# lavaman131/dinov2.cpp

Hardware: AMD Instinct MI355X
Metric: images/sec (518x518), ViT-L/14 fp16 (higher is better)
Workload: dtype f16; 1 GPU; dinov2-large (ViT-L/14, 4 registers) f16 GGUF, 518x518, batch=32 per GPU, classify head, random-init weights; global_batch=32, parallelism=dp1

## Files before the change

dinov2.cpp_amd/csrc/gemm4.hip:

```cpp
#include <cstdio>
#include <type_traits>
#include <utility>

#include "device_types.h"
#include "gemm_epilogue.h"
#include "kernels.h"

namespace dinov2 {

template <int... Is, class F>
static __device__ __forceinline__ void static_for_impl(std::integer_sequence<int, Is...>, F&& f) {
    (f(std::integral_constant<int, Is>{}), ...);
}
template <int N, class F>
static __device__ __forceinline__ void static_for(F&& f) {
    static_for_impl(std::make_integer_sequence<int, N>{}, static_cast<F&&>(f));
}

#define DINO4_MFMA_F16(ACC, W, X) asm volatile("v_mfma_f32_16x16x32_f16 %0, %1, %2, %0" : "+a"(ACC) : "v"(W), "v"(X))
#define DINO4_MFMA_F16_Z(ACC, W, X) asm volatile("v_mfma_f32_16x16x32_f16 %0, %1, %2, 0" : "=a"(ACC) : "v"(W), "v"(X))
#define DINO4_MFMA_BF16(ACC, W, X) asm volatile("v_mfma_f32_16x16x32_bf16 %0, %1, %2, %0" : "+a"(ACC) : "v"(W), "v"(X))
#define DINO4_MFMA_BF16_Z(ACC, W, X) asm volatile("v_mfma_f32_16x16x32_bf16 %0, %1, %2, 0" : "=a"(ACC) : "v"(W), "v"(X))
#define DINO4_DSR(DST, ADDR, OFF) asm volatile("ds_read_b128 %0, %1 offset:%2" : "=v"(DST) : "v"(ADDR), "n"(OFF))
#define DINO4_GLDS(VOFF, SBASE, LDSBASE, IMM)                                                                                   \
    asm volatile("s_add_u32 m0, %2, %3\n\ts_nop 0\n\tglobal_load_lds_dwordx4 %0, %1" ::"v"(VOFF), "s"(SBASE), "s"(LDSBASE), "n"(IMM) \
                 : "memory", "scc")

__device__ unsigned long long g_clk4[CLK_SLOTS * 4];
hipError_t gemm4_clock_probe_read(unsigned long long* out) {
    return hipMemcpyFromSymbol(out, HIP_SYMBOL(g_clk4), sizeof(unsigned long long) * CLK_SLOTS * 4);
}

constexpr int G4_PA = 39, G4_PB = 103;

#ifdef DINO_GEMM4_PROF
__device__ unsigned long long g_gemm4_prof[256 * 4];
#define DINO4_GP_DECL unsigned long long gp_t = 0, gp_r = 0, gp_acc[4] = {0, 0, 0, 0};
#define DINO4_GP_START { gp_t = __builtin_readcyclecounter(); gp_r = __builtin_amdgcn_s_memrealtime(); }
#define DINO4_GP(i) { const unsigned long long t__ = __builtin_readcyclecounter(); gp_acc[i] += t__ - gp_t; gp_t = t__; }
#define DINO4_GP_TILE { gp_acc[2] += 1; const unsigned long long r__ = __builtin_amdgcn_s_memrealtime(); gp_acc[3] += r__ - gp_r; gp_r = r__; }
#define DINO4_GP_FLUSH if (threadIdx.x == 0) for (int i__ = 0; i__ < 4; ++i__) g_gemm4_prof[blockIdx.x * 4 + i__] += gp_acc[i__];
#else
#define DINO4_GP_DECL
#define DINO4_GP_START
#define DINO4_GP(i)
#define DINO4_GP_TILE
#define DINO4_GP_FLUSH
#endif

template <typename T, int EPI, int NI>
static __device__ __forceinline__ void gemm4_body(const GemmArgs& p, char* smem) {
#pragma clang fp contract(off)
    using E = Elem<T>;
    using vec4 = typename E::vec4;
    constexpr bool F16 = std::is_same<T, _Float16>::value;
    constexpr bool LNC = EPI == EPI_QKV_LN || EPI == EPI_GELU_LN || EPI == EPI_SWIGLU_LN;
    constexpr int EB = EPI == EPI_RESID_LN ? EPI_RESID : EPI == EPI_QKV_LN ? EPI_QKV : EPI == EPI_GELU_LN ? EPI_GELU : EPI == EPI_SWIGLU_LN ? EPI_SWIGLU : EPI;
    constexpr int BM = 32 * NI, BN = 256;
    constexpr int NP = NI + 8;
    constexpr int SP = NI <= 4 ? 4 : 8;
    constexpr int G4_NPRE = G4_PA / SP + 1;
    constexpr int NSLOT = 128 / SP - G4_NPRE;
    constexpr int NPOST = NP < NSLOT ? NP : NSLOT;
    constexpr int NBS = (G4_PB - SP * G4_NPRE) / SP + 1;
    constexpr int G4_NB = NBS < NPOST ? NBS : NPOST;
    static_assert(NP - NPOST <= G4_NPRE, "staging schedule");

    DINO4_GP_DECL
    int tid = threadIdx.x;
    asm volatile("" : "+v"(tid));
    const int lane = tid & 63;
    const int wid = __builtin_amdgcn_readfirstlane(tid >> 6);
    const int wr = wid >> 1, wc = wid & 1;
    const int M = p.M, N = p.N, K = p.K;
    const bool nt_out = p.nt_out != 0;
    const unsigned lda2 = (unsigned)(p.lda ? p.lda : K) * 2u, ldw2 = (unsigned)(p.ldw ? p.ldw : K) * 2u;
    const int ntn = N / BN, ntm = (M + BM - 1) / BM;
    const int ntiles = ntn * ntm;
    const int nk = K / 64;

    const int xcd = blockIdx.x & 7, bidx = blockIdx.x >> 3;
    const int nb_x = ((int)gridDim.x >> 3) + (xcd < ((int)gridDim.x & 7) ? 1 : 0);
    const int tq = ntiles >> 3, tr = ntiles & 7;
    const int chunk0 = xcd < tr ? xcd * (tq + 1) : tr * (tq + 1) + (xcd - tr) * tq;
    const int chunkn = tq + (xcd < tr ? 1 : 0);
    constexpr int GM = 8;
    auto tile_mn = [&](int lid, int& m0, int& n0) {
        const int g = lid / (GM * ntn), r = lid - g * (GM * ntn);
        const int gm = ntm - g * GM < GM ? ntm - g * GM : GM;
        const int n = r / gm, mi = r - n * gm;
        m0 = (g * GM + mi) * BM;
        n0 = n * BN;
    };

    unsigned so[NP];
    auto piece_off = [&](int pc, int m0, int n0) -> unsigned {
        const bool isw = pc >= 2 * NI || (pc & 1);
        const int rb = pc >= 2 * NI ? pc - NI : pc >> 1;
        int pl = lane;
        if constexpr (LNC) asm volatile("" : "+v"(pl));
        const int r = (isw ? 64 : 8 * NI) * wid + 8 * rb + (pl >> 3);
        const int ch = (pl & 7) ^ ((r >> 1) & 7);
        if (isw) return (unsigned)(n0 + r) * ldw2 + ch * 16;
        int gm = m0 + r;
        gm = gm < M ? gm : M - 1;
        return (unsigned)gm * lda2 + ch * 16;
    };
    const unsigned lds0 = (unsigned)(uintptr_t)(DINO_LDS_AS char*)smem;
    const unsigned ldsx = lds0 + (unsigned)wid * (NI * 1024u), ldsw = lds0 + 65536u + (unsigned)wid * 8192u;

    const int fr = lane & 15, kq = lane >> 4, sw = (fr >> 1) & 7;
    unsigned xa[2], wa[2];
#pragma unroll
    for (int ks = 0; ks < 2; ++ks) {
        const unsigned ch = (unsigned)(((ks * 4 + kq) ^ sw) << 4);
        xa[ks] = lds0 + (unsigned)((wr * (16 * NI) + fr) * 128) + ch;
        wa[ks] = lds0 + 65536u + (unsigned)((wc * 128 + fr) * 128) + ch;
    }

    f32x4 acc[NI][8];
    u32x4 Px[NI], Pw[8], Qx[NI], Qw[8];

    const char* const Ab = (const char*)p.A;
    const char* const Wb = (const char*)p.W;

#define DINO4_PIECE(PC, KT, BUF)                                                                                            \
    {                                                                                                                       \
        constexpr int pc__ = (PC);                                                                                          \
        constexpr bool isw__ = pc__ >= 2 * NI || (pc__ & 1);                                                                \
        constexpr int rb__ = pc__ >= 2 * NI ? pc__ - NI : pc__ >> 1;                                                        \
        if constexpr (isw__) {                                                                                              \
            DINO4_GLDS(so[pc__], Wb + (size_t)(KT) * 128, ldsw, (BUF) * 32768 + rb__ * 1024);                               \
        } else {                                                                                                            \
            DINO4_GLDS(so[pc__], Ab + (size_t)(KT) * 128, ldsx, (BUF) * 32768 + rb__ * 1024);                               \
        }                                                                                                                   \
    }

    auto ktile = [&acc, &Px, &Pw, &Qx, &Qw, &xa, &wa, &so, &ldsx, &ldsw, Ab, Wb](auto bc, auto firstc, int kt_pre, bool pre_on, auto&& at_a,
                                                                                int kt_post, bool post_on, bool do_readp) {
        static_for<128>([&acc, &Px, &Pw, &Qx, &Qw, &xa, &wa, &so, &ldsx, &ldsw, Ab, Wb, &kt_pre, &pre_on, &at_a, &kt_post, &post_on, &do_readp,
                         bc, firstc](auto mc) {
            constexpr int m = decltype(mc)::value;
            constexpr int b = decltype(bc)::value;
            constexpr bool FIRST = decltype(firstc)::value;
            constexpr int ks = m >> 6, j = (m >> 3) & 7, i = m & 7;
            if constexpr (i < NI) {
                if constexpr (ks == 0) {
                    if constexpr (FIRST) {
                        if constexpr (F16) DINO4_MFMA_F16_Z(acc[i][j], Pw[j], Px[i]);
                        else DINO4_MFMA_BF16_Z(acc[i][j], Pw[j], Px[i]);
                    } else {
                        if constexpr (F16) DINO4_MFMA_F16(acc[i][j], Pw[j], Px[i]);
                        else DINO4_MFMA_BF16(acc[i][j], Pw[j], Px[i]);
                    }
                } else {
                    if constexpr (F16) DINO4_MFMA_F16(acc[i][j], Qw[j], Qx[i]);
                    else DINO4_MFMA_BF16(acc[i][j], Qw[j], Qx[i]);
                }
            }
            if constexpr (m % 2 == 0 && m / 2 < 8 + NI) {
                constexpr int q = m / 2;
                if constexpr (q < 8) DINO4_DSR(Qw[q], wa[1], q * 2048 + b * 32768);
                else DINO4_DSR(Qx[q - 8], xa[1], (q - 8) * 2048 + b * 32768);
            }
            if constexpr (m % SP == 0) {
                constexpr int k = m / SP;
                if constexpr (k < G4_NPRE) {
                    if constexpr (NPOST + k < NP) {
                        if (pre_on) DINO4_PIECE(NPOST + k, kt_pre, b ^ 1)
                    }
                } else if constexpr (k - G4_NPRE < NPOST) {
                    if (post_on) DINO4_PIECE(k - G4_NPRE, kt_post, b)
                }
            }
            if constexpr (m == G4_PA) {
                asm volatile("s_waitcnt lgkmcnt(0)" ::: "memory");
                asm volatile("s_barrier" ::: "memory");
                at_a();
            }
            if constexpr (m == G4_PB) {
                if (post_on) asm volatile("s_waitcnt vmcnt(%0)" ::"n"(G4_NB) : "memory");
                else asm volatile("s_waitcnt vmcnt(0)" ::: "memory");
                asm volatile("s_barrier" ::: "memory");
            }
            if constexpr (m > G4_PB && m <= G4_PB + 8 + NI) {
                constexpr int q = m - G4_PB - 1;
                if (do_readp) {
                    if constexpr (q < 8) DINO4_DSR(Pw[q], wa[0], q * 2048 + (b ^ 1) * 32768);
                    else DINO4_DSR(Px[q - 8], xa[0], (q - 8) * 2048 + (b ^ 1) * 32768);
                }
            }
        });
        asm volatile("s_waitcnt lgkmcnt(0)" ::: "memory");
    };
    static_assert(2 * (8 + 8) - 2 < G4_PA && G4_PB + 16 <= 127, "fragment reads fit their windows");

    using T0 = std::integral_constant<int, 0>;
    using T1 = std::integral_constant<int, 1>;
    using TT = std::integral_constant<bool, true>;
    using TF = std::integral_constant<bool, false>;
    auto nop = [] {};

    constexpr int LNH = !LNC ? 0 : NI > 4 ? 2 : 1;
    float st_r[LNH ? LNH : 1], st_n[LNH ? LNH : 1];
    const int ln_gs = p.ln_gs;
    const float ln_inv_h = 1.0f / (float)K;
    auto ln_row_of = [&](int m0_, int h) {
        int ll = lane;
        asm volatile("" : "+v"(ll));
        int rl = h * 64 + ll;
        rl = rl < 16 * NI ? rl : 16 * NI - 1;
        const int row = m0_ + wr * (16 * NI) + rl;
        return row < M ? row : M - 1;
    };

    if (bidx < chunkn) {
        int pm0, pn0;
        tile_mn(chunk0 + bidx, pm0, pn0);
#pragma unroll
        for (int pc = 0; pc < NP; ++pc) so[pc] = piece_off(pc, pm0, pn0);
        asm volatile("s_waitcnt vmcnt(0) lgkmcnt(0)\n\ts_barrier" ::: "memory");
        LnRaw lraw[LNH ? LNH : 1], lraw1[LNH ? LNH : 1];
        if constexpr (LNC) {
#pragma unroll
            for (int h = 0; h < LNH; ++h) {
                ln_row_load<0>(p.stats, ln_row_of(pm0, h), ln_gs, lraw[h]);
                if (ln_gs > 12) ln_row_load<1>(p.stats, ln_row_of(pm0, h), ln_gs, lraw1[h]);
            }
        }
        static_for<NP>([&so, &ldsx, &ldsw, Ab, Wb](auto pcc) { DINO4_PIECE(decltype(pcc)::value, 0, 0) });
        static_for<NPOST>([&so, &ldsx, &ldsw, Ab, Wb](auto pcc) { DINO4_PIECE(decltype(pcc)::value, 1, 1) });
        asm volatile("s_waitcnt vmcnt(%0)" ::"n"(NPOST) : "memory");
        asm volatile("s_barrier" ::: "memory");
        static_for<8 + NI>([&Px, &Pw, &xa, &wa](auto qc) {
            constexpr int q = decltype(qc)::value;
            if constexpr (q < 8) DINO4_DSR(Pw[q], wa[0], q * 2048);
            else DINO4_DSR(Px[q - 8], xa[0], (q - 8) * 2048);
        });
        asm volatile("s_waitcnt lgkmcnt(0)" ::: "memory");
        if constexpr (LNC) {
#pragma unroll
            for (int h = 0; h < LNH; ++h) {
                LnAcc la;
                ln_row_add<0>(lraw[h], la);
                if (ln_gs > 12) ln_row_add<1>(lraw1[h], la);
                ln_row_finish(la, ln_inv_h, p.ln_eps, st_r[h], st_n[h]);
            }
        }
    }
    for (int tix = bidx; tix < chunkn; tix += nb_x) {
        int m0, n0;
        tile_mn(chunk0 + tix, m0, n0);
        const bool has_next = tix + nb_x < chunkn;
        DINO4_GP_START

        ktile(T0{}, TT{}, 1, true, nop, 2, true, true);
        ktile(T1{}, TF{}, 2, true, nop, 3, true, true);
        for (int t = 2; t < nk - 2; t += 2) {
            ktile(T0{}, TF{}, t + 1, true, nop, t + 2, true, true);
            ktile(T1{}, TF{}, t + 2, true, nop, t + 3, true, true);
        }
        int nm0 = 0, nn0 = 0;
        if (has_next) tile_mn(chunk0 + tix + nb_x, nm0, nn0);
        ktile(T0{}, TF{}, nk - 1, true,
              [&] {
                  if (has_next) {
                      if constexpr (LNC) {
                          if (m0 + BM <= M && nm0 + BM <= M) {
                              const unsigned dx = (unsigned)(nm0 - m0) * lda2, dw = (unsigned)(nn0 - n0) * ldw2;
#pragma unroll
                              for (int pc = 0; pc < NP; ++pc) so[pc] += (pc >= 2 * NI || (pc & 1)) ? dw : dx;
                          } else {
#pragma unroll
                              for (int pc = 0; pc < NP; ++pc) so[pc] = piece_off(pc, nm0, nn0);
                          }
                      } else {
#pragma unroll
                          for (int pc = 0; pc < NP; ++pc) so[pc] = piece_off(pc, nm0, nn0);
                      }
                  }
              },
              0, has_next, true);
        float4 lnsc = make_float4(0.f, 0.f, 0.f, 0.f);
        if constexpr (LNC) {
            int ll = lane;
            asm volatile("" : "+v"(ll));
            lnsc = *(const float4*)((ll < 32 ? p.ln_s : p.ln_c) + n0 + wc * 128 + 4 * (ll & 31));
        }
        ktile(T1{}, TF{}, 0, has_next, nop, 1, has_next, has_next && !LNC);
        asm volatile("s_nop 15\n\ts_nop 7" ::: "memory");
        static_for<NI * 8>([&acc](auto ic) { asm volatile("" : "+a"(acc[decltype(ic)::value / 8][decltype(ic)::value % 8])); });
        DINO4_GP(0)

        int el = lane;
        asm volatile("" : "+v"(el));
        const int er = el & 15, eq = el >> 4;
        char* const ep = smem + 131072 + wid * 8192;
        const int mbase = m0 + wr * (16 * NI);
        float cu_r[LNH ? LNH : 1], cu_n[LNH ? LNH : 1];
        if constexpr (LNC) {
#pragma unroll
            for (int h = 0; h < LNH; ++h) {
                cu_r[h] = st_r[h];
                cu_n[h] = st_n[h];
            }
        }
#define DINO4_ACC(Q_, B_, I_, J_) acc[((Q_)*4 + (I_)) < NI ? ((Q_)*4 + (I_)) : 0][cg * 4 + (B_)*2 + (J_)]
#pragma unroll
        for (int cg = 0; cg < 2; ++cg) {
            const int nw0 = n0 + wc * 128 + cg * 64;
            const int ncol = nw0 + 4 * eq;
            float4 bs[2][2];
            if constexpr (!LNC && EPI != EPI_RESID_LN) {
#pragma unroll
                for (int b = 0; b < 2; ++b)
#pragma unroll
                    for (int j = 0; j < 2; ++j)
                        bs[b][j] = p.bias ? *(const float4*)(p.bias + ncol + b * 32 + j * 16) : make_float4(0.f, 0.f, 0.f, 0.f);
            }
            float4 lsv[LNC ? 2 : 1][2], lcv[LNC ? 2 : 1][2];
            if constexpr (LNC) {
#pragma unroll
                for (int b = 0; b < 2; ++b)
#pragma unroll
                    for (int j = 0; j < 2; ++j) {
                        const int f = cg * 16 + b * 8 + j * 4 + eq;
                        lsv[b][j] = make_float4(__shfl(lnsc.x, f), __shfl(lnsc.y, f), __shfl(lnsc.z, f), __shfl(lnsc.w, f));
                        lcv[b][j] = make_float4(__shfl(lnsc.x, 32 + f), __shfl(lnsc.y, 32 + f), __shfl(lnsc.z, 32 + f), __shfl(lnsc.w, 32 + f));
                    }
            }
            LnRaw lraw;
            LnAcc lacc;
            const bool ln_next = LNC && cg < LNH && has_next;
            if constexpr (LNC) {
                if (ln_next) ln_row_load<0>(p.stats, ln_row_of(nm0, cg), ln_gs, lraw);
            }

            if constexpr (EB == EPI_QKV || EB == EPI_GELU || EB == EPI_SWIGLU) {
                const float qs = (EB == EPI_QKV && nw0 < p.qcols) ? p.qscale : 1.0f;
                constexpr int BN_ = EB == EPI_SWIGLU ? 1 : 2;
#pragma unroll
                for (int q = 0; q < 2; ++q) {
                    if constexpr (LNC) {
                        if (q == 1 && ln_next) {
                            ln_row_add<0>(lraw, lacc);
                            if (ln_gs > 12) ln_row_load<1>(p.stats, ln_row_of(nm0, cg), ln_gs, lraw);
                        }
                    }
                    if (q * 4 >= NI) continue;
                    float lnr[LNC ? 4 : 1], lnn[LNC ? 4 : 1];
                    if constexpr (LNC) {
#pragma unroll
                        for (int i = 0; i < 4; ++i) {
                            lnr[i] = __shfl(cu_r[q < LNH ? q : 0], 16 * i + er);
                            lnn[i] = __shfl(cu_n[q < LNH ? q : 0], 16 * i + er);
                        }
                    }
#pragma unroll
                    for (int b = 0; b < BN_; ++b)
#pragma unroll
                        for (int j = 0; j < 2; ++j) {
                            float4 bbv, b2v, sbv = make_float4(0.f, 0.f, 0.f, 0.f), s2v = make_float4(0.f, 0.f, 0.f, 0.f);
                            if constexpr (LNC) {
                                sbv = lsv[b][j];
                                bbv = lcv[b][j];
                                b2v = lcv[1][j];
                                s2v = lsv[1][j];
                            } else {
                                bbv = bs[b][j];
                                b2v = bs[1][j];
                            }
                            const float bb[4] = {bbv.x, bbv.y, bbv.z, bbv.w};
                            const float b2[4] = {b2v.x, b2v.y, b2v.z, b2v.w};
                            const float sb[4] = {sbv.x, sbv.y, sbv.z, sbv.w};
                            const float s2[4] = {s2v.x, s2v.y, s2v.z, s2v.w};
#pragma unroll
                            for (int i = 0; i < 4; ++i) {
                                if (q * 4 + i >= NI) continue;
                                const int ir = i;
                                vec4 o;
                                if constexpr (EB == EPI_GELU) {
#pragma unroll
                                    for (int e2 = 0; e2 < 2; ++e2) {
                                        const f32x2 a2 = {DINO4_ACC(q, b, i, j)[2 * e2], DINO4_ACC(q, b, i, j)[2 * e2 + 1]};
                                        f32x2 v;
                                        if constexpr (LNC) v = epi_ln(lnr[LNC ? ir : 0], lnn[LNC ? ir : 0], a2, f32x2{sb[2 * e2], sb[2 * e2 + 1]}, f32x2{bb[2 * e2], bb[2 * e2 + 1]});
                                        else v = epi_bias(a2, f32x2{bb[2 * e2], bb[2 * e2 + 1]});
                                        const f32x2 g = epi_gelu(v);
                                        o[2 * e2] = E::from_f32(g[0]);
                                        o[2 * e2 + 1] = E::from_f32(g[1]);
                                    }
                                } else {
#pragma unroll
                                    for (int e = 0; e < 4; ++e) {
                                        float v;
                                        if constexpr (LNC) v = epi_ln(lnr[LNC ? ir : 0], lnn[LNC ? ir : 0], DINO4_ACC(q, b, i, j)[e], sb[e], bb[e]);
                                        else v = epi_bias(DINO4_ACC(q, b, i, j)[e], bb[e]);
                                        if constexpr (EB == EPI_QKV) {
                                            o[e] = epi_qkv<E>(v, qs);
                                        } else {
                                            float h2;
                                            if constexpr (LNC) h2 = epi_ln_raw(lnr[LNC ? ir : 0], lnn[LNC ? ir : 0], DINO4_ACC(q, 1, i, j)[e], s2[e], b2[e]);
                                            else h2 = epi_bias_raw(DINO4_ACC(q, 1, i, j)[e], b2[e]);
                                            o[e] = E::from_f32(epi_swiglu(v, h2));
                                        }
                                    }
                                }
                                const int row = i * 16 + er;
                                const int slot = (4 * b + 2 * j + (eq >> 1)) ^ (row & 7);
                                *(vec4*)(ep + row * 128 + slot * 16 + (eq & 1) * 8) = o;
                            }
                        }
                    __builtin_amdgcn_wave_barrier();
                    if constexpr (EB == EPI_SWIGLU) {
                        const int hid0 = (nw0 >> 6) * 32;
#pragma unroll
                        for (int it = 0; it < 4; ++it) {
                            const int row = it * 16 + (el >> 2), slot = el & 3;
                            const u32x4 v = *(const u32x4*)(ep + row * 128 + ((slot ^ (row & 7)) << 4));
                            const int m = mbase + q * 64 + row;
                            if (m < M && (NI == 8 || q * 64 + row < 16 * NI))
                                DINO_EPI_ST16((u32x4*)((T*)p.out + (size_t)m * p.ldo + hid0 + slot * 8), v, nt_out);
                        }
                    } else {
#pragma unroll
                        for (int it = 0; it < 8; ++it) {
                            const int row = it * 8 + (el >> 3), slot = el & 7;
                            const u32x4 v = *(const u32x4*)(ep + row * 128 + ((slot ^ (row & 7)) << 4));
                            const int trw = q * 64 + row;
                            const int m = mbase + trw;
                            if (m < M && (NI == 8 || trw < 16 * NI))
                                DINO_EPI_ST16((u32x4*)((T*)p.out + (size_t)m * p.ldo + nw0 + slot * 8), v, nt_out);
                        }
                    }
                    __builtin_amdgcn_wave_barrier();
                }
            } else {
            }
            if constexpr (LNC) {
                if (ln_next) {
                    if (ln_gs > 12) ln_row_add<1>(lraw, lacc);
                    ln_row_finish(lacc, ln_inv_h, p.ln_eps, st_r[cg < LNH ? cg : 0], st_n[cg < LNH ? cg : 0]);
                }
            }
        }
        if constexpr (EPI == EPI_RESID || EPI == EPI_PLAIN_F32) {
            constexpr int PF = 3;
            float4 add[8][8];
            auto pass_cols = [&](int ps8, int& nb, int& q) {
                const int cg = ps8 >> 2, b = (ps8 >> 1) & 1;
                q = ps8 & 1;
                nb = n0 + wc * 128 + cg * 64 + b * 32 + (el & 7) * 4;
            };
            auto issue_loads = [&](int ps8) {
                if constexpr (EPI == EPI_RESID) {
                    int nb, q;
                    pass_cols(ps8, nb, q);
#pragma unroll
                    for (int it = 0; it < 8; ++it) {
                        int m = mbase + q * 64 + it * 8 + (el >> 3);
                        m = m < M ? m : M - 1;
                        add[ps8][it] = *(const float4*)((const float*)p.out + (size_t)m * p.ldo + nb);
                    }
                }
            };
#pragma unroll
            for (int ps8 = 0; ps8 < PF; ++ps8) issue_loads(ps8);
#pragma unroll
            for (int ps8 = 0; ps8 < 8; ++ps8) {
                const int cg = ps8 >> 2, b = (ps8 >> 1) & 1, q = ps8 & 1;
                if (q * 4 >= NI) continue;
                asm volatile("" : "+v"(el));
                const int ncol = n0 + wc * 128 + cg * 64 + 4 * (el >> 4);
                const int nb = n0 + wc * 128 + cg * 64 + b * 32 + (el & 7) * 4;
#pragma unroll
                for (int j = 0; j < 2; ++j) {
                    float4 ls = make_float4(1.f, 1.f, 1.f, 1.f);
                    if constexpr (EPI == EPI_RESID) ls = *(const float4*)(p.aux + ncol + b * 32 + j * 16);
                    const float4 b4 = p.bias ? *(const float4*)(p.bias + ncol + b * 32 + j * 16) : make_float4(0.f, 0.f, 0.f, 0.f);
#pragma unroll
                    for (int i = 0; i < 4; ++i) {
                        if (q * 4 + i >= NI) continue;
                        const int row = i * 16 + (el & 15);
                        const int slot = (4 * j + (el >> 4)) ^ (row & 7);
                        *(float4*)(ep + row * 128 + slot * 16) = epi_layerscale(DINO4_ACC(q, b, i, j), b4, ls);
                    }
                }
                if (ps8 + PF < 8) issue_loads(ps8 + PF);
                __builtin_amdgcn_wave_barrier();
#pragma unroll
                for (int it = 0; it < 8; ++it) {
                    const int row = it * 8 + (el >> 3), slot = el & 7;
                    float4 v = *(const float4*)(ep + row * 128 + ((slot ^ (row & 7)) << 4));
                    if constexpr (EPI == EPI_RESID) v = epi_residual(v, add[ps8][it]);
                    const int m = mbase + q * 64 + row;
                    if (m < M && (NI == 8 || q * 64 + row < 16 * NI)) *(float4*)((float*)p.out + (size_t)m * p.ldo + nb) = v;
                }
                __builtin_amdgcn_wave_barrier();
            }
        }
        if constexpr (EPI == EPI_RESID_LN) {
            constexpr int PF = 2;
            float4 add[8][8];
            auto pass_of = [&](int ps8, int& cg, int& q, int& ih) {
                cg = ps8 >> 2;
                q = (ps8 >> 1) & 1;
                ih = ps8 & 1;
            };
            auto pass_live = [&](int ps8) {
                const int q = (ps8 >> 1) & 1, ih = ps8 & 1;
                return q * 4 + ih * 2 < NI;
            };
            auto issue_loads = [&](int ps8) {
                int cg, q, ih;
                pass_of(ps8, cg, q, ih);
                const int nb = n0 + wc * 128 + cg * 64 + (el & 15) * 4;
#pragma unroll
                for (int it = 0; it < 8; ++it) {
                    int m = mbase + q * 64 + ih * 32 + it * 4 + (el >> 4);
                    m = m < M ? m : M - 1;
                    add[ps8][it] = *(const float4*)((const float*)p.out + (size_t)m * p.ldo + nb);
                }
            };
            int issued = 0;
#pragma unroll
            for (int ps8 = 0; ps8 < 8; ++ps8)
                if (pass_live(ps8) && issued < PF) {
                    issue_loads(ps8);
                    ++issued;
                }
#pragma unroll
            for (int ps8 = 0; ps8 < 8; ++ps8) {
                if (!pass_live(ps8)) continue;
                int cg, q, ih;
                pass_of(ps8, cg, q, ih);
                asm volatile("" : "+v"(el));
                const int ncol = n0 + wc * 128 + cg * 64 + 4 * (el >> 4);
                const int nb = n0 + wc * 128 + cg * 64 + (el & 15) * 4;
#pragma unroll
                for (int b = 0; b < 2; ++b)
#pragma unroll
                    for (int j = 0; j < 2; ++j) {
                        const float4 ls = *(const float4*)(p.aux + ncol + b * 32 + j * 16);
                        const float4 b4 = p.bias ? *(const float4*)(p.bias + ncol + b * 32 + j * 16) : make_float4(0.f, 0.f, 0.f, 0.f);
#pragma unroll
                        for (int ii = 0; ii < 2; ++ii) {
                            if (q * 4 + ih * 2 + ii >= NI) continue;
                            const int row = ii * 16 + (el & 15);
                            const int slot = (b * 8 + j * 4 + (el >> 4)) ^ (row & 15);
                            *(float4*)(ep + row * 256 + slot * 16) = epi_layerscale(DINO4_ACC(q, b, ih * 2 + ii, j), b4, ls);
                        }
                    }
                const float4 gam = *(const float4*)(p.ln_gamma + nb);
                {
                    int ahead = 0;
#pragma unroll
                    for (int nx = ps8 + 1; nx < 8; ++nx)
                        if (pass_live(nx) && ++ahead == PF) issue_loads(nx);
                }
                __builtin_amdgcn_wave_barrier();
                float ssum = 0.f, ssq = 0.f;
#pragma unroll
                for (int it = 0; it < 8; ++it) {
                    const int row = it * 4 + (el >> 4), slot = el & 15;
                    float4 v = *(const float4*)(ep + row * 256 + ((slot ^ (row & 15)) << 4));
                    v = epi_residual(v, add[ps8][it]);
                    const int rl = q * 64 + ih * 32 + row;
                    const int m = mbase + rl;
                    const bool live = m < M && (NI == 8 || rl < 16 * NI);
                    if (live) *(float4*)((float*)p.out + (size_t)m * p.ldo + nb) = v;
                    const vec4 og = epi_xg<E>(v, gam);
                    if (live) *(vec4*)((T*)p.xg + (size_t)m * p.ldo + nb) = og;
                    float s4, q4;
                    ln_leaf4(v.x, v.y, v.z, v.w, s4, q4);
                    s4 += dpp_f32<0xB1>(s4);
                    q4 += dpp_f32<0xB1>(q4);
                    s4 += dpp_f32<0x4E>(s4);
                    q4 += dpp_f32<0x4E>(q4);
                    s4 += dpp_f32<0x141>(s4);
                    q4 += dpp_f32<0x141>(q4);
                    s4 += dpp_f32<0x140>(s4);
                    q4 += dpp_f32<0x140>(q4);
                    if ((el & 15) == it) {
                        ssum = s4;
                        ssq = q4;
                    }
                }
                {
                    const int rl = q * 64 + ih * 32 + (el & 15) * 4 + (el >> 4);
                    const int m = mbase + rl;
                    if ((el & 15) < 8 && m < M && (NI == 8 || rl < 16 * NI))
                        *(float2*)(p.stats + ((size_t)m * p.ln_gs + ((n0 + wc * 128 + cg * 64) >> 6)) * 2) = make_float2(ssum, ssq);
                }
                __builtin_amdgcn_wave_barrier();
            }
        }
#undef DINO4_ACC
        if constexpr (LNC) {
            if (has_next) {
                static_for<8 + NI>([&Px, &Pw, &xa, &wa](auto qc) {
                    constexpr int q = decltype(qc)::value;
                    if constexpr (q < 8) DINO4_DSR(Pw[q], wa[0], q * 2048);
                    else DINO4_DSR(Px[q - 8], xa[0], (q - 8) * 2048);
                });
                asm volatile("s_waitcnt lgkmcnt(0)" ::: "memory");
            }
        }
        DINO4_GP(1)
        DINO4_GP_TILE
    }
    DINO4_GP_FLUSH
#undef DINO4_PIECE
}

template <typename T, int EPI, int NI>
__global__ __launch_bounds__(256) void gemm4_kernel(GemmArgs p) {
    extern __shared__ __attribute__((aligned(16))) char smem[];
    DINO_CLK_BEGIN()
    gemm4_body<T, EPI, NI>(p, smem);
    DINO_CLK_END(g_clk4, p.clk_slot)
}

template <typename T, int EPI>
__global__ __launch_bounds__(256) void gemm4_mixed_kernel(GemmArgs p, GemmArgs q) {
    extern __shared__ __attribute__((aligned(16))) char smem[];
    DINO_CLK_BEGIN()
    gemm4_body<T, EPI, 8>(p, smem);
    gemm4_body<T, EPI, 6>(q, smem);
    DINO_CLK_END(g_clk4, p.clk_slot)
}

constexpr size_t G4_LDS = 163840;

#ifdef DINO_GEMM4_PROF
static void gemm4_prof_dump(const char* what, int epi, int nblocks) {
    static unsigned long long h[256 * 4], z[256 * 4];
    (void)hipDeviceSynchronize();
    (void)hipMemcpyFromSymbol(h, HIP_SYMBOL(g_gemm4_prof), sizeof h);
    (void)hipMemcpyToSymbol(HIP_SYMBOL(g_gemm4_prof), z, sizeof z);
    double a[4] = {0, 0, 0, 0};
    for (int b = 0; b < nblocks; ++b)
        for (int i = 0; i < 4; ++i) a[i] += (double)h[b * 4 + i];
    const double t = a[2] > 0 ? a[2] : 1;
    fprintf(stderr, "gemm4_prof %s epi %d: per tile (wave 0): K loop %.0f cycles, epilogue %.0f cycles, %.2f us in all (%.2f tiles per workgroup) -> clock %.3f GHz\n", what, epi,
            a[0] / t, a[1] / t, a[3] / t * 0.01, a[2] / nblocks, (a[0] + a[1]) / (a[3] * 10.0));
}
#endif

#define DINO4_EPIS(X) X(EPI_QKV) X(EPI_RESID) X(EPI_GELU) X(EPI_SWIGLU) X(EPI_PLAIN_F32) X(EPI_RESID_LN) X(EPI_QKV_LN) X(EPI_GELU_LN) X(EPI_SWIGLU_LN)
constexpr bool gemm4_short_epi(int e) { return e != EPI_RESID && e != EPI_PLAIN_F32; }
template <typename T, int NI>
static GemmKernelFn kernel4(int epi) {
    switch (epi) {
#define DINO_X(E)                                                                        \
    case E:                                                                              \
        if constexpr (NI == 8 || gemm4_short_epi(E)) return gemm4_kernel<T, E, NI>; \
        else return nullptr;
        DINO4_EPIS(DINO_X)
#undef DINO_X
        default: return nullptr;
    }
}
template <typename T>
static GemmKernelFn2 kernel4_mixed(int epi) {
    switch (epi) {
#define DINO_X(E) case E: return gemm4_mixed_kernel<T, E>;
        DINO4_EPIS(DINO_X)
#undef DINO_X
        default: return nullptr;
    }
}

bool gemm4_ok(Epilogue epi, int N, int K) { return epi != EPI_PATCH && N % 256 == 0 && K % 128 == 0 && K >= 256; }
template <typename T>
static GemmKernelFn kernel4_ni(int ni, int epi) {
    return ni == 8 ? kernel4<T, 8>(epi) : ni == 2 ? kernel4<T, 2>(epi) : ni == 3 ? kernel4<T, 3>(epi) : ni == 4 ? kernel4<T, 4>(epi) : nullptr;
}
hipError_t launch_gemm4(DType dt, Epilogue epi, const GemmArgs& a, int ni, hipStream_t st) {
    const GemmKernelFn k = dt == DT_F16 ? kernel4_ni<_Float16>(ni, epi) : kernel4_ni<__bf16>(ni, epi);
    if (!k) return hipErrorInvalidValue;
    const int tiles = (a.N / 256) * ((a.M + 32 * ni - 1) / (32 * ni));
    if (ni != 8 && tiles > 256) return hipErrorInvalidValue;
    hipLaunchKernelGGL(k, dim3(tiles < 256 ? tiles : 256), dim3(256), G4_LDS, st, a);
#ifdef DINO_GEMM4_PROF
    if (ni == 8) gemm4_prof_dump("plain launch", (int)epi, tiles < 256 ? tiles : 256);
#endif
    return hipGetLastError();
}
hipError_t launch_gemm4_mixed(DType dt, Epilogue epi, const GemmArgs& a, const GemmArgs& b, hipStream_t st) {
    const GemmKernelFn2 k = dt == DT_F16 ? kernel4_mixed<_Float16>(epi) : kernel4_mixed<__bf16>(epi);
    if (!k) return hipErrorInvalidValue;
    hipLaunchKernelGGL(k, dim3(256), dim3(256), G4_LDS, st, a, b);
#ifdef DINO_GEMM4_PROF
    gemm4_prof_dump("mixed launch", (int)epi, 256);
#endif
    return hipGetLastError();
}
template <typename T>
static hipError_t attr4_t() {
    hipError_t e = hipSuccess;
    for (int epi = 0; epi < EPI_COUNT && e == hipSuccess; ++epi) {
        e = gemm_raise_lds((const void*)kernel4<T, 8>(epi), G4_LDS);
        if (e == hipSuccess) e = gemm_raise_lds((const void*)kernel4_mixed<T>(epi), G4_LDS);
        if (e == hipSuccess) e = gemm_raise_lds((const void*)kernel4<T, 2>(epi), G4_LDS);
        if (e == hipSuccess) e = gemm_raise_lds((const void*)kernel4<T, 3>(epi), G4_LDS);
        if (e == hipSuccess) e = gemm_raise_lds((const void*)kernel4<T, 4>(epi), G4_LDS);
    }
    return e;
}

hipError_t gemm4_init() {
    const hipError_t e = attr4_t<_Float16>();
    return e == hipSuccess ? attr4_t<__bf16>() : e;
}

}
```

Measured before the change: 935.5 images/sec.

## Software-pipeline non-LN GEMM epilogue with double-buffered LDS half-tiles and early bias loads

```diff
diff --git a/dinov2.cpp_amd/csrc/gemm4.hip b/dinov2.cpp_amd/csrc/gemm4.hip
--- a/dinov2.cpp_amd/csrc/gemm4.hip
+++ b/dinov2.cpp_amd/csrc/gemm4.hip
@@ -34,18 +34,26 @@
 constexpr int G4_PA = 39, G4_PB = 103;
 
 #ifdef DINO_GEMM4_PROF
-__device__ unsigned long long g_gemm4_prof[256 * 4];
-#define DINO4_GP_DECL unsigned long long gp_t = 0, gp_r = 0, gp_acc[4] = {0, 0, 0, 0};
+constexpr int G4_NPROF = 8;
+__device__ unsigned long long g_gemm4_prof[256 * G4_NPROF];
+#define DINO4_GP_DECL unsigned long long gp_t = 0, gp_r = 0, gp_acc[G4_NPROF] = {0, 0, 0, 0, 0, 0, 0, 0};
 #define DINO4_GP_START { gp_t = __builtin_readcyclecounter(); gp_r = __builtin_amdgcn_s_memrealtime(); }
 #define DINO4_GP(i) { const unsigned long long t__ = __builtin_readcyclecounter(); gp_acc[i] += t__ - gp_t; gp_t = t__; }
 #define DINO4_GP_TILE { gp_acc[2] += 1; const unsigned long long r__ = __builtin_amdgcn_s_memrealtime(); gp_acc[3] += r__ - gp_r; gp_r = r__; }
-#define DINO4_GP_FLUSH if (threadIdx.x == 0) for (int i__ = 0; i__ < 4; ++i__) g_gemm4_prof[blockIdx.x * 4 + i__] += gp_acc[i__];
+#define DINO4_GP_FLUSH if (threadIdx.x == 0) for (int i__ = 0; i__ < G4_NPROF; ++i__) g_gemm4_prof[blockIdx.x * G4_NPROF + i__] += gp_acc[i__];
 #else
 #define DINO4_GP_DECL
 #define DINO4_GP_START
 #define DINO4_GP(i)
 #define DINO4_GP_TILE
 #define DINO4_GP_FLUSH
+#endif
+#if defined(DINO_GEMM4_PROF) && DINO_GEMM4_PROF >= 2
+constexpr bool G4_PHASED = true;
+#define DINO4_GP_PHASE(i) { __builtin_amdgcn_sched_barrier(0); DINO4_GP(i) __builtin_amdgcn_sched_barrier(0); }
+#else
+constexpr bool G4_PHASED = false;
+#define DINO4_GP_PHASE(i)
 #endif
 
 template <typename T, int EPI, int NI>
@@ -281,6 +289,21 @@
                   }
               },
               0, has_next, true);
+        constexpr bool EPI2 = EB == EPI_QKV || EB == EPI_GELU || EB == EPI_SWIGLU;
+        constexpr bool BIAS_AHEAD = EPI2 && !LNC;
+        float4 bsa[BIAS_AHEAD ? 2 : 1][2][2];
+        if constexpr (BIAS_AHEAD) {
+            int ll = lane;
+            asm volatile("" : "+v"(ll));
+            const float* const bp = p.bias + n0 + wc * 128 + 4 * (ll >> 4);
+#pragma unroll
+            for (int cg = 0; cg < 2; ++cg)
+#pragma unroll
+                for (int b = 0; b < 2; ++b)
+#pragma unroll
+                    for (int j = 0; j < 2; ++j)
+                        bsa[cg][b][j] = p.bias ? *(const float4*)(bp + cg * 64 + b * 32 + j * 16) : make_float4(0.f, 0.f, 0.f, 0.f);
+        }
         float4 lnsc = make_float4(0.f, 0.f, 0.f, 0.f);
         if constexpr (LNC) {
             int ll = lane;
@@ -305,18 +328,73 @@
                 cu_n[h] = st_n[h];
             }
         }
+        auto epi_block = [](const f32x4& a, const f32x4& ag, const float4& bbv, const float4& b2v, const float4& sbv, const float4& s2v, float lr, float lnm, float qs) -> vec4 {
+            const float bb[4] = {bbv.x, bbv.y, bbv.z, bbv.w};
+            const float b2[4] = {b2v.x, b2v.y, b2v.z, b2v.w};
+            const float sb[4] = {sbv.x, sbv.y, sbv.z, sbv.w};
+            const float s2[4] = {s2v.x, s2v.y, s2v.z, s2v.w};
+            vec4 o;
+            if constexpr (EB == EPI_GELU) {
+#pragma unroll
+                for (int e2 = 0; e2 < 2; ++e2) {
+                    const f32x2 a2 = {a[2 * e2], a[2 * e2 + 1]};
+                    f32x2 v;
+                    if constexpr (LNC) v = epi_ln(lr, lnm, a2, f32x2{sb[2 * e2], sb[2 * e2 + 1]}, f32x2{bb[2 * e2], bb[2 * e2 + 1]});
+                    else v = epi_bias(a2, f32x2{bb[2 * e2], bb[2 * e2 + 1]});
+                    const f32x2 g = epi_gelu(v);
+                    o[2 * e2] = E::from_f32(g[0]);
+                    o[2 * e2 + 1] = E::from_f32(g[1]);
+                }
+            } else {
+#pragma unroll
+                for (int e = 0; e < 4; ++e) {
+                    float v;
+                    if constexpr (LNC) v = epi_ln(lr, lnm, a[e], sb[e], bb[e]);
+                    else v = epi_bias(a[e], bb[e]);
+                    if constexpr (EB == EPI_QKV) {
+                        o[e] = epi_qkv<E>(v, qs);
+                    } else {
+                        float h2;
+                        if constexpr (LNC) h2 = epi_ln_raw(lr, lnm, ag[e], s2[e], b2[e]);
+                        else h2 = epi_bias_raw(ag[e], b2[e]);
+                        o[e] = E::from_f32(epi_swiglu(v, h2));
+                    }
+                }
+            }
+            return o;
+        };
+        constexpr int LPR = EB == EPI_SWIGLU ? 4 : 8, LSH = EB == EPI_SWIGLU ? 2 : 3;
+        auto lines_read = [&](auto rows_c, const char* eh, u32x4* rv) {
+            constexpr int ROWS = decltype(rows_c)::value;
+#pragma unroll
+            for (int it = 0; it < ROWS * LPR / 64; ++it) {
+                const int row = it * (64 / LPR) + (el >> LSH), slot = el & (LPR - 1);
+                rv[it] = *(const u32x4*)(eh + row * 128 + ((slot ^ (row & 7)) << 4));
+            }
+        };
+        auto lines_store = [&](auto rows_c, int trw0, int nw0, const u32x4* rv) {
+            constexpr int ROWS = decltype(rows_c)::value;
+            const int c0 = EB == EPI_SWIGLU ? (nw0 >> 6) * 32 : nw0;
+#pragma unroll
+            for (int it = 0; it < ROWS * LPR / 64; ++it) {
+                const int row = it * (64 / LPR) + (el >> LSH), slot = el & (LPR - 1);
+                const int trw = trw0 + row;
+                const int m = mbase + trw;
+                if (m < M && (NI == 8 || trw < 16 * NI))
+                    DINO_EPI_ST16((u32x4*)((T*)p.out + (size_t)m * p.ldo + c0 + slot * 8), rv[it], nt_out);
+            }
+        };
+        constexpr bool PIPE2 = EPI2 && !LNC && !G4_PHASED;
 #define DINO4_ACC(Q_, B_, I_, J_) acc[((Q_)*4 + (I_)) < NI ? ((Q_)*4 + (I_)) : 0][cg * 4 + (B_)*2 + (J_)]
 #pragma unroll
         for (int cg = 0; cg < 2; ++cg) {
             const int nw0 = n0 + wc * 128 + cg * 64;
-            const int ncol = nw0 + 4 * eq;
             float4 bs[2][2];
-            if constexpr (!LNC && EPI != EPI_RESID_LN) {
+            if constexpr (BIAS_AHEAD) {
 #pragma unroll
                 for (int b = 0; b < 2; ++b)
 #pragma unroll
-                    for (int j = 0; j < 2; ++j)
-                        bs[b][j] = p.bias ? *(const float4*)(p.bias + ncol + b * 32 + j * 16) : make_float4(0.f, 0.f, 0.f, 0.f);
+                    for (int j = 0; j < 2; ++j) bs[b][j] = bsa[cg][b][j];
             }
             float4 lsv[LNC ? 2 : 1][2], lcv[LNC ? 2 : 1][2];
             if constexpr (LNC) {
@@ -336,9 +414,11 @@
                 if (ln_next) ln_row_load<0>(p.stats, ln_row_of(nm0, cg), ln_gs, lraw);
             }
 
-            if constexpr (EB == EPI_QKV || EB == EPI_GELU || EB == EPI_SWIGLU) {
+            if constexpr (EPI2 && !PIPE2) {
                 const float qs = (EB == EPI_QKV && nw0 < p.qcols) ? p.qscale : 1.0f;
                 constexpr int BN_ = EB == EPI_SWIGLU ? 1 : 2;
+                [[maybe_unused]] const float4 zero4 = make_float4(0.f, 0.f, 0.f, 0.f);
+                using R64 = std::integral_constant<int, 64>;
 #pragma unroll
                 for (int q = 0; q < 2; ++q) {
                     if constexpr (LNC) {
@@ -356,56 +436,67 @@
                             lnn[i] = __shfl(cu_n[q < LNH ? q : 0], 16 * i + er);
                         }
                     }
+                    if constexpr (G4_PHASED && !LNC) {
+                        u32x4 rv[8];
+#pragma unroll
+                        for (int b = 0; b < 2; ++b)
+#pragma unroll
+                            for (int j = 0; j < 2; ++j) asm volatile("" : "+v"(bs[b][j].x), "+v"(bs[b][j].y), "+v"(bs[b][j].z), "+v"(bs[b][j].w));
+                        DINO4_GP_PHASE(7)
+                        f32x4 ra[2][2][4];
+#pragma unroll
+                        for (int b = 0; b < 2; ++b)
+#pragma unroll
+                            for (int j = 0; j < 2; ++j)
+#pragma unroll
+                                for (int i = 0; i < 4; ++i) {
+                                    ra[b][j][i] = DINO4_ACC(q, b, i, j);
+                                    asm volatile("" : "+v"(ra[b][j][i]));
+                                }
+                        DINO4_GP_PHASE(4)
+                        typedef unsigned u32x2_ __attribute__((ext_vector_type(2)));
+                        u32x2_ ov[BN_][2][4];
+#pragma unroll
+                        for (int b = 0; b < BN_; ++b)
+#pragma unroll
+                            for (int j = 0; j < 2; ++j)
+#pragma unroll
+                                for (int i = 0; i < 4; ++i) {
+                                    ov[b][j][i] = __builtin_bit_cast(u32x2_, epi_block(ra[b][j][i], ra[1][j][i], bs[b][j], bs[1][j], zero4, zero4, 0.f, 0.f, qs));
+                                    asm volatile("" : "+v"(ov[b][j][i]));
+                                }
+                        DINO4_GP_PHASE(5)
+#pragma unroll
+                        for (int b = 0; b < BN_; ++b)
+#pragma unroll
+                            for (int j = 0; j < 2; ++j)
+#pragma unroll
+                                for (int i = 0; i < 4; ++i) {
+                                    if (q * 4 + i >= NI) continue;
+                                    const int row = i * 16 + er;
+                                    const int slot = (4 * b + 2 * j + (eq >> 1)) ^ (row & 7);
+                                    *(u32x2_*)(ep + row * 128 + slot * 16 + (eq & 1) * 8) = ov[b][j][i];
+                                }
+                        __builtin_amdgcn_wave_barrier();
+                        lines_read(R64{}, ep, rv);
+                        asm volatile("s_waitcnt lgkmcnt(0)" ::: "memory");
+#pragma unroll
+                        for (int it = 0; it < 8; ++it) asm volatile("" : "+v"(rv[it]));
+                        DINO4_GP_PHASE(6)
+                        lines_store(R64{}, q * 64, nw0, rv);
+                        __builtin_amdgcn_wave_barrier();
+                        continue;
+                    }
 #pragma unroll
                     for (int b = 0; b < BN_; ++b)
 #pragma unroll
                         for (int j = 0; j < 2; ++j) {
-                            float4 bbv, b2v, sbv = make_float4(0.f, 0.f, 0.f, 0.f), s2v = make_float4(0.f, 0.f, 0.f, 0.f);
-                            if constexpr (LNC) {
-                                sbv = lsv[b][j];
-                                bbv = lcv[b][j];
-                                b2v = lcv[1][j];
-                                s2v = lsv[1][j];
-                            } else {
-                                bbv = bs[b][j];
-                                b2v = bs[1][j];
-                            }
-                            const float bb[4] = {bbv.x, bbv.y, bbv.z, bbv.w};
-                            const float b2[4] = {b2v.x, b2v.y, b2v.z, b2v.w};
-                            const float sb[4] = {sbv.x, sbv.y, sbv.z, sbv.w};
-                            const float s2[4] = {s2v.x, s2v.y, s2v.z, s2v.w};
 #pragma unroll
                             for (int i = 0; i < 4; ++i) {
                                 if (q * 4 + i >= NI) continue;
-                                const int ir = i;
                                 vec4 o;
-                                if constexpr (EB == EPI_GELU) {
-#pragma unroll
-                                    for (int e2 = 0; e2 < 2; ++e2) {
-                                        const f32x2 a2 = {DINO4_ACC(q, b, i, j)[2 * e2], DINO4_ACC(q, b, i, j)[2 * e2 + 1]};
-                                        f32x2 v;
-                                        if constexpr (LNC) v = epi_ln(lnr[LNC ? ir : 0], lnn[LNC ? ir : 0], a2, f32x2{sb[2 * e2], sb[2 * e2 + 1]}, f32x2{bb[2 * e2], bb[2 * e2 + 1]});
-                                        else v = epi_bias(a2, f32x2{bb[2 * e2], bb[2 * e2 + 1]});
-                                        const f32x2 g = epi_gelu(v);
-                                        o[2 * e2] = E::from_f32(g[0]);
-                                        o[2 * e2 + 1] = E::from_f32(g[1]);
-                                    }
-                                } else {
-#pragma unroll
-                                    for (int e = 0; e < 4; ++e) {
-                                        float v;
-                                        if constexpr (LNC) v = epi_ln(lnr[LNC ? ir : 0], lnn[LNC ? ir : 0], DINO4_ACC(q, b, i, j)[e], sb[e], bb[e]);
-                                        else v = epi_bias(DINO4_ACC(q, b, i, j)[e], bb[e]);
-                                        if constexpr (EB == EPI_QKV) {
-                                            o[e] = epi_qkv<E>(v, qs);
-                                        } else {
-                                            float h2;
-                                            if constexpr (LNC) h2 = epi_ln_raw(lnr[LNC ? ir : 0], lnn[LNC ? ir : 0], DINO4_ACC(q, 1, i, j)[e], s2[e], b2[e]);
-                                            else h2 = epi_bias_raw(DINO4_ACC(q, 1, i, j)[e], b2[e]);
-                                            o[e] = E::from_f32(epi_swiglu(v, h2));
-                                        }
-                                    }
-                                }
+                                if constexpr (LNC) o = epi_block(DINO4_ACC(q, b, i, j), DINO4_ACC(q, 1, i, j), lcv[b][j], lcv[1][j], lsv[b][j], lsv[1][j], lnr[LNC ? i : 0], lnn[LNC ? i : 0], qs);
+                                else o = epi_block(DINO4_ACC(q, b, i, j), DINO4_ACC(q, 1, i, j), bs[b][j], bs[1][j], zero4, zero4, 0.f, 0.f, qs);
                                 const int row = i * 16 + er;
                                 const int slot = (4 * b + 2 * j + (eq >> 1)) ^ (row & 7);
                                 *(vec4*)(ep + row * 128 + slot * 16 + (eq & 1) * 8) = o;
@@ -442,6 +533,63 @@
                     if (ln_gs > 12) ln_row_add<1>(lraw, lacc);
                     ln_row_finish(lacc, ln_inv_h, p.ln_eps, st_r[cg < LNH ? cg : 0], st_n[cg < LNH ? cg : 0]);
                 }
+            }
+        }
+        if constexpr (G4_PHASED && EPI2 && !LNC) {
+            DINO4_GP_PHASE(7)
+        }
+        if constexpr (PIPE2) {
+            constexpr int BN_ = EB == EPI_SWIGLU ? 1 : 2;
+            using R32 = std::integral_constant<int, 32>;
+            const float4 zero4 = make_float4(0.f, 0.f, 0.f, 0.f);
+            u32x4 rv[4];
+            int prev = -1, nlive = 0;
+#pragma unroll
+            for (int sp = 0; sp <= 8; ++sp) {
+                const int cg = (sp >> 2) & 1, q = (sp >> 1) & 1, ih = sp & 1;
+                const bool live = sp < 8 && q * 4 + ih * 2 < NI;
+                if (sp < 8 && !live) continue;
+                const int pcg = (prev >> 2) & 1, pq = (prev >> 1) & 1, pih = prev & 1;
+                if (prev >= 0) {
+                    lines_read(R32{}, ep + ((nlive - 1) & 1) * 4096, rv);
+                    __builtin_amdgcn_sched_barrier(0);
+                }
+                vec4 o[BN_][2][2];
+                float qs = 1.0f;
+                if (live) {
+                    const int nw0 = n0 + wc * 128 + cg * 64;
+                    qs = (EB == EPI_QKV && nw0 < p.qcols) ? p.qscale : 1.0f;
+#pragma unroll
+                    for (int b = 0; b < BN_; ++b)
+#pragma unroll
+                        for (int j = 0; j < 2; ++j)
+#pragma unroll
+                            for (int ii = 0; ii < 2; ++ii) {
+                                const int i = ih * 2 + ii;
+                                o[b][j][ii] = epi_block(DINO4_ACC(q, b, i, j), DINO4_ACC(q, 1, i, j), bsa[cg][b][j], bsa[cg][1][j], zero4, zero4, 0.f, 0.f, qs);
+                            }
+                }
+                if (prev >= 0) {
+                    asm volatile("s_waitcnt lgkmcnt(0)" ::: "memory");
+                    lines_store(R32{}, pq * 64 + pih * 32, n0 + wc * 128 + pcg * 64, rv);
+                }
+                if (live) {
+                    char* const eh = ep + (nlive & 1) * 4096;
+#pragma unroll
+                    for (int b = 0; b < BN_; ++b)
+#pragma unroll
+                        for (int j = 0; j < 2; ++j)
+#pragma unroll
+                            for (int ii = 0; ii < 2; ++ii) {
+                                if (q * 4 + ih * 2 + ii >= NI) continue;
+                                const int row = ii * 16 + er;
+                                const int slot = (4 * b + 2 * j + (eq >> 1)) ^ (row & 7);
+                                *(vec4*)(eh + row * 128 + slot * 16 + (eq & 1) * 8) = o[b][j][ii];
+                            }
+                }
+                __builtin_amdgcn_wave_barrier();
+                prev = live ? sp : -1;
+                nlive += live ? 1 : 0;
             }
         }
         if constexpr (EPI == EPI_RESID || EPI == EPI_PLAIN_F32) {
@@ -634,16 +782,20 @@
 
 #ifdef DINO_GEMM4_PROF
 static void gemm4_prof_dump(const char* what, int epi, int nblocks) {
-    static unsigned long long h[256 * 4], z[256 * 4];
+    static unsigned long long h[256 * G4_NPROF], z[256 * G4_NPROF];
     (void)hipDeviceSynchronize();
     (void)hipMemcpyFromSymbol(h, HIP_SYMBOL(g_gemm4_prof), sizeof h);
     (void)hipMemcpyToSymbol(HIP_SYMBOL(g_gemm4_prof), z, sizeof z);
-    double a[4] = {0, 0, 0, 0};
+    double a[G4_NPROF] = {0, 0, 0, 0, 0, 0, 0, 0};
     for (int b = 0; b < nblocks; ++b)
-        for (int i = 0; i < 4; ++i) a[i] += (double)h[b * 4 + i];
+        for (int i = 0; i < G4_NPROF; ++i) a[i] += (double)h[b * G4_NPROF + i];
     const double t = a[2] > 0 ? a[2] : 1;
+    const double epil = a[1] + a[4] + a[5] + a[6] + a[7];
     fprintf(stderr, "gemm4_prof %s epi %d: per tile (wave 0): K loop %.0f cycles, epilogue %.0f cycles, %.2f us in all (%.2f tiles per workgroup) -> clock %.3f GHz\n", what, epi,
-            a[0] / t, a[1] / t, a[3] / t * 0.01, a[2] / nblocks, (a[0] + a[1]) / (a[3] * 10.0));
+            a[0] / t, epil / t, a[3] / t * 0.01, a[2] / nblocks, (a[0] + epil) / (a[3] * 10.0));
+    if (G4_PHASED)
+        fprintf(stderr, "gemm4_prof %s epi %d: epilogue phases per tile: read-out %.0f, arithmetic %.0f, LDS transpose %.0f, stores + next wait %.0f, rest %.0f cycles\n", what, epi,
+                a[4] / t, a[5] / t, a[6] / t, a[7] / t, a[1] / t);
 }
 #endif
 
```

After: 933.2 images/sec. No clear change (-0.3%).
